# elcritch/figdraw

Hardware: AMD Instinct MI355X
Metric: Mpixels/s composited @3840x2160, 300 SDF rects+shadows; % HBM roofline (higher is better)
Workload: dtype f32 (blur taps: u8 x f16 -> f32 MFMA); 1 GPU; S300@4K: renderlist_100 scene at 3840x2160, 300 shadowed SDF rects + full-frame and 360x240 2-pass Gaussian backdrop blur(18) (BASELINE.json configs[2]); draws=707, phases=3, blur_nodes=2, fragments=41088819, parallelism=single GPU, frames_in_flight_per_gpu=4, walk_pool_threads=7, walk_pool_threads_default=7

## Files before the change

figdraw_amd/context.py:

```python
from __future__ import annotations

import ctypes as C
import os
import subprocess
from typing import Optional

import numpy as np

from . import scene as S

_HERE = os.path.dirname(os.path.abspath(__file__))
LIB_PATH = os.path.join(_HERE, "libfigdraw_hip.so")
_lib = None

_F4 = C.c_float * 4
_F2 = C.c_float * 2
_COL4 = S.CColor * 4


class FigdrawHipError(RuntimeError):
    def __init__(self, code: int, msg: str):
        super().__init__(f"[{code}] {msg}")
        self.code = code

# ... 376 lines not shown
    L.fdh_set_ui_scale.argtypes = [vp, C.c_float]
    L.fdh_render_frame.argtypes = [vp, vp, C.c_float, C.c_float, C.c_int, _F4]
    L.fdh_set_stripe.argtypes = [vp, C.c_int, C.c_int]
    L.fdh_set_blur_route.argtypes = [vp, C.c_int]
    L.fdh_set_cull.argtypes = [vp, C.c_int]
    L.fdh_culled_draws.argtypes = [vp, C.POINTER(C.c_int64)]
    L.fdh_set_walk_threads.argtypes = [vp, C.c_int]
    L.fdh_debug_host_times.argtypes = [vp, C.POINTER(C.c_int64)]
    L.fdh_walk_stats.argtypes = [vp, C.POINTER(C.c_int), C.POINTER(C.c_int64)]
    L.fdh_stripe_rows.argtypes = [C.c_int, C.c_int, C.c_int, C.POINTER(C.c_int), C.POINTER(C.c_int)]
    L.fdh_comm_unique_id.argtypes = [C.c_char_p]
    L.fdh_comm_init.argtypes = [vp, C.c_char_p, C.c_int, C.c_int]
    L.fdh_comm_destroy.argtypes = [vp]
    L.fdh_comm_share.argtypes = [vp, vp]
    L.fdh_gather_stripes.argtypes = [vp, C.c_int, vp]
    L.fdh_gather_frames.argtypes = [vp, C.c_int, C.POINTER(vp)]
    L.fdh_replay.argtypes = [vp, C.c_int]
    L.fdh_replay_async.argtypes = [vp, C.c_int]
    L.fdh_replay_timed.argtypes = [vp, C.c_int, C.POINTER(C.c_float)]
    L.fdh_profile.argtypes = [vp, C.c_int]
    L.fdh_get_frame_stats.argtypes = [vp, C.POINTER(FrameStats)]
    if hasattr(L, "fdh_block_wave_bins"):
        L.fdh_block_wave_bins.argtypes = [vp, C.POINTER(C.c_int)]
    if hasattr(L, "fdh_set_damage_tracking"):
        L.fdh_set_damage_tracking.argtypes = [vp, C.c_int]
        L.fdh_damage_bins.argtypes = [vp, vp, C.c_int, C.POINTER(C.c_int), C.POINTER(C.c_int), C.POINTER(C.c_int)]
        L.fdh_damage_changed_bins.argtypes = [vp, vp, C.c_int, C.POINTER(C.c_int), C.POINTER(C.c_int), C.POINTER(C.c_int)]
        L.fdh_damage_closure.argtypes = [vp, C.c_int, C.c_int, vp, vp, C.c_int, vp]
    if hasattr(L, "fdh_set_damage_readback"):
        L.fdh_set_damage_readback.argtypes = [vp, C.c_int]
        L.fdh_read_damage.argtypes = [vp, C.POINTER(vp), C.POINTER(vp), C.POINTER(C.c_int), C.POINTER(C.c_int), C.POINTER(C.c_int), C.POINTER(C.c_int)]
        L.fdh_read_damage_into.argtypes = [vp, vp, C.c_int64, C.c_int, C.c_int, C.POINTER(C.c_int)]
        L.fdh_apply_damage.argtypes = [vp, C.c_int64, C.c_int, C.c_int, vp, vp, C.c_int]
    if hasattr(L, "fdh_read_damage_coded"):
        L.fdh_read_damage_coded.argtypes = [vp, C.POINTER(vp), C.POINTER(vp), C.POINTER(C.c_int), C.POINTER(C.c_int64), C.POINTER(C.c_int), C.POINTER(C.c_int),
                                            C.POINTER(C.c_int)]
        L.fdh_decode_damage.argtypes = [vp, C.c_int64, C.c_int, C.c_int, vp, C.c_int, vp, C.c_int64]
        L.fdh_coded_damage_bound.argtypes = [C.c_int, C.c_int]
        L.fdh_coded_damage_bound.restype = C.c_int64
    if hasattr(L, "fdh_set_damage_exact"):
        L.fdh_set_damage_exact.argtypes = [vp, C.c_int]
        L.fdh_damage_exact_stats.argtypes = [vp, C.POINTER(C.c_int), C.POINTER(C.c_int), C.POINTER(C.c_int)]
    if hasattr(L, "fdh_read_damage_moved"):
        L.fdh_read_damage_moved.argtypes = [vp, vp, C.c_int, C.POINTER(vp), C.POINTER(vp), C.POINTER(C.c_int), C.POINTER(C.c_int64), C.POINTER(C.c_int),
                                            C.POINTER(C.c_int), C.POINTER(C.c_int), C.POINTER(C.c_int)]
        L.fdh_decode_damage_moved.argtypes = [vp, C.c_int64, C.c_int, C.c_int, vp, C.c_int, vp, C.c_int64]
# ... 775 lines not shown
    def gather_frames(self, dst_rank: int = 0, dst_ptrs=None):
        arr = (C.c_void_p * len(dst_ptrs))(*dst_ptrs) if dst_ptrs else None
        self._ck(self.L.fdh_gather_frames(self.h, int(dst_rank), arr))

    def replay(self, times: int = 1):
        self._ck(self.L.fdh_replay(self.h, int(times)))

    def replay_async(self, times: int = 1):
        self._ck(self.L.fdh_replay_async(self.h, int(times)))

    def replay_timed(self, times: int):
        out = (C.c_float * int(times))()
        self._ck(self.L.fdh_replay_timed(self.h, int(times), out))
        return np.array(out, dtype=np.float32)

    def profile(self, times: int = 1):
        self._ck(self.L.fdh_profile(self.h, int(times)))

    def frame_stats(self) -> FrameStats:
        st = FrameStats()
        self._ck(self.L.fdh_get_frame_stats(self.h, C.byref(st)))
        return st

    def block_wave_bins(self) -> int:
        n = C.c_int(0)
        self._ck(self.L.fdh_block_wave_bins(self.h, C.byref(n)))
        return n.value
```

figdraw_amd/csrc/fdh_capi.cpp:

```cpp
#include <string>

#include "fdh_context.h"
#include "fdh_damage.h"
#include "../../include/figdraw_hip_damage.h"
#include "../../include/figdraw_hip_pick.h"
#include "../../include/figdraw_hip_readback.h"
#include "../../include/figdraw_hip_stream.h"
#include "../../include/figdraw_hip_exact.h"
#include "../../include_schedule/figdraw_hip_schedule.h"
#include "../../include_readback/figdraw_hip_moves.h"
#include "../../include_glyphs/figdraw_hip_glyphs.h"
#include "../../include_glyphs/figdraw_hip_coverage.h"
#include "../../include_glyphs/figdraw_hip_cubic.h"
#include "../../include_glyphs/figdraw_hip_image_sdf.h"
#include "../../include_glyphs/figdraw_hip_device_image.h"
#include "../../include_glyphs/figdraw_hip_device_images.h"
#include "../../include_glyphs/figdraw_hip_video_frame.h"
#include "../../include_glyphs/figdraw_hip_atlas.h"
#include "../../include_video/figdraw_hip_video_out.h"
#include "../../include_video/figdraw_hip_video_planar.h"
#include "../../include_video/figdraw_hip_video_422.h"
#include "../../include_video/figdraw_hip_video_alpha.h"

using fdh::Context;
// ... 482 lines not shown
    if (!out_ns) throw fdh::Error(FDH_ERR_INVALID, "null output");
    for (int i = 0; i < 12; i++) out_ns[i] = C(c)->host_ns_[i];
  });
}
int fdh_set_walk_threads(FdhContext* c, int n) { return guard([&] { C(c)->set_walk_threads(n); }); }
int fdh_walk_stats(FdhContext* c, int* threads, int64_t* parallel_groups) {
  return guard([&] {
    if (threads) *threads = C(c)->walk_threads();
    if (parallel_groups) *parallel_groups = C(c)->parallel_groups();
  });
}
int fdh_culled_draws(FdhContext* c, int64_t* out) {
  return guard([&] {
    if (!out) throw fdh::Error(FDH_ERR_INVALID, "null output");
    *out = C(c)->culled_draws();
  });
}
int fdh_replay(FdhContext* c, int times) { return guard([&] { C(c)->replay(times); }); }
int fdh_replay_async(FdhContext* c, int times) { return guard([&] { C(c)->replay_async(times); }); }
int fdh_replay_timed(FdhContext* c, int times, float* ms_out) { return guard([&] { C(c)->replay_timed(times, ms_out); }); }
int fdh_profile(FdhContext* c, int times) { return guard([&] { C(c)->profile(times); }); }
int fdh_get_frame_stats(FdhContext* c, FdhFrameStats* out) { return guard([&] { C(c)->frame_stats(out); }); }
int fdh_block_wave_bins(FdhContext* c, int* out) { return guard([&] { *out = C(c)->block_wave_bins(); }); }

}
```

figdraw_amd/csrc/fdh_context.cpp:

```cpp
#include "fdh_context.h"
#include "fdh_host.h"
#include "fdh_walkpool.h"

#include <chrono>

#include <algorithm>
#include <cmath>
#include <cstdio>
#include <cstring>

namespace fdh {

void hip_check(hipError_t e, const char* what) {
  if (e != hipSuccess) throw Error(FDH_ERR_HIP, std::string(what) + ": " + hipGetErrorString(e));
}

void poison_fresh(void* p, size_t bytes) {
#if defined(FDH_POISON)
  if (!p || !bytes) return;
  (void)hipMemset(p, FDH_POISON, bytes);
  (void)hipDeviceSynchronize();
#else
  (void)p; (void)bytes;
#endif
// ... 427 lines not shown
  const bool big = ph.blur == J.big_blur;
  const int vy0 = std::max(j.y0, row_lo), vy1 = std::min(j.y1, row_hi);
  if (vy1 <= vy0 || j.x1 <= j.x0) return cur;
  BlurParams bp;
  bp.W = J.W; bp.H = J.H; bp.pitch = J.W;
  bp.taps = j.taps;
  bp.node_pixels = (long long)(j.x1 - j.x0) * (j.y1 - j.y0);
  bp.fuse_draw = -1;
  bp.mx_w = (size_t)ph.blur < J.mx_w_h.size() ? J.mx_w_h[ph.blur] : nullptr;
  bp.opaque = J.opaque ? 1 : 0;
  bp.x0 = j.x0; bp.x1 = j.x1; bp.y0 = vy0; bp.y1 = vy1;
  if ((size_t)ph.blur < J.blur_fused.size() && J.blur_fused[ph.blur]) {
    uint32_t* other = cur == fb_ ? alt_ : fb_;
    bp.src = cur; bp.dst = other;
    bp.fuse_draw = j.fuse_draw;
    span_begin(kSpanBlurFused);
    const bool done = launch_blur_fused(stream_, bp, J.mx_w_v[ph.blur], J.dv.recs, J.dv.exts);
    span_end();
    if (!done) throw Error(FDH_ERR_HIP, "fused blur: no kernel for this filter width (blur_fused_supported out of step with the launcher)");
    return other;
  }
  if (j.fuse_draw < 0 && J.latency_routes && blur_one_kernel_ok(j.x1 - j.x0, j.y1 - j.y0, j.taps.reach)) {
    bp.src = cur; bp.dst = backdrop_;
    span_begin(big ? kSpanBigBlurV : kSpanBlurV);
    launch_blur_small(stream_, bp);
    span_end();
    return cur;
  }
  bp.src = cur; bp.dst = blur_tmp_;
  bp.y0 = std::max(0, vy0 - j.taps.reach); bp.y1 = std::min(J.H, vy1 + j.taps.reach);
  const bool guard = partial && j.fuse_draw >= 0;
  if (guard) damage_.guard(stream_, J, ph.blur, false, cur, vy0, vy1);
  span_begin(big ? kSpanBigBlurH : kSpanBlurH);
  launch_blur_h(stream_, bp);
  span_end();
  bp.src = blur_tmp_; bp.dst = j.fuse_draw >= 0 ? cur : backdrop_;
  bp.mx_w = (size_t)ph.blur < J.mx_w_v.size() ? J.mx_w_v[ph.blur] : nullptr;
  bp.fuse_draw = j.fuse_draw;
  bp.y0 = vy0; bp.y1 = vy1;
  span_begin(big ? kSpanBigBlurV : kSpanBlurV);
  launch_blur_v(stream_, bp, J.dv.recs, J.dv.exts);
  span_end();
  if (guard) damage_.guard(stream_, J, ph.blur, true, cur, vy0, vy1);
  return cur;
}

// ... 271 lines not shown
```

figdraw_amd/csrc/fdh_context.h:

```cpp
#pragma once
#include <hip/hip_runtime.h>

#include <algorithm>
#include <atomic>
#include <chrono>
#include <condition_variable>
#include <cstdint>
#include <cstdlib>
#include <cstring>
#include <exception>
#include <memory>
#include <mutex>
#include <stdexcept>
#include <string>
#include <thread>
#include <unordered_map>
#include <vector>

#include "../../include/figdraw_hip.h"
#include "../../include/figdraw_hip_pick.h"
#include "../../include/figdraw_hip_readback.h"
#include "../../include/figdraw_hip_stream.h"
#include "fdh_kernels.h"
#include "fdh_plain.h"
// ... 115 lines not shown
  void set_pick_tag(int32_t z, int32_t id) { set_tag(PickTag{z, id}); }
  void pick_points(const float* xy, int n, int threshold, uint32_t flags, int max_hits, FdhPickHit* out, int* counts);
  void pick_region(int x, int y, int w, int h, int threshold, uint32_t flags, int32_t* out_draw);
  void pick_draw_tags(int32_t* zlevels, int32_t* ids, int cap, int* n);
  void set_cull(int mode) { frame_env_.cull_mode = mode < 0 ? 0 : (mode > 2 ? 2 : mode); }
  int64_t culled_draws() const { return culled_total_; }
  void set_walk_threads(int n) { walk_threads_ = n < 0 ? -1 : (n > 64 ? 64 : n); }
  int walk_threads() const;
  int64_t parallel_groups() const { return parallel_groups_; }
  struct GroupCuts { int first_item = -1, n = 0; std::vector<int> cut; std::vector<float> cost; uint64_t used = 0; };
  std::vector<GroupCuts>& group_cuts() { return group_cuts_; }
  void count_parallel_group() { parallel_groups_++; }
  bool may_fork() const { return env_.frame_begun && !call_log_.on(); }
  RecordedFrame& frame() { return frame_; }
  void reopen_piece() { set_phase_floor(frame_.open_piece()); }
  Recorder& pool_recorder(int slot);
  void use_device_here() const;
  void set_blur_route(int route) { blur_route_ = route < 0 ? -1 : (route ? 1 : 0); }
  void replay(int times);
  void replay_timed(int times, float* ms_out);
  void replay_async(int times);
  void profile(int times);
  int block_wave_bins() { drain(); return block_wave_bins_; }
  void frame_stats(FdhFrameStats* out) { drain(); *out = stats_; out->ms_host_launch = launch_ms_.load(std::memory_order_relaxed); }
  void flush() { drain(); }

 private:
  void release_device_state();
  void make_rect_image() override;
  void blur_node(const DrawRec& quad, const float rect[4], float blur_radius) override;
  uint32_t resolve_lcd(uint32_t flags) const {
    if (!(flags & FDH_GLYPH_LCD_CONTEXT) || (flags & FDH_GLYPH_MTSDF)) return flags;
    return (flags & ~(uint32_t)(FDH_GLYPH_LCD_FILTER | FDH_GLYPH_LCD_CONTEXT)) | (text_lcd_filtering_ ? FDH_GLYPH_LCD_FILTER : 0u);
  }
  struct FoldGuard {
    BinRec* br = nullptr;
    BBox box{0, 0, 0, 0};
    FoldGuard() = default;
    FoldGuard(FoldGuard&& o) noexcept : br(o.br), box(o.box) { o.br = nullptr; }
    FoldGuard(const FoldGuard&) = delete;
    FoldGuard& operator=(const FoldGuard&) = delete;
    ~FoldGuard() { if (br) br->box = box; }
  };

  void prepare(LaunchJob& J);
  void describe_frame(LaunchJob& J);
// ... 93 lines not shown
  bool pick_on_ = false;
  void pick_check(const char* who, int threshold, uint32_t flags);
  DeviceBuf<uint8_t> d_pick_, d_pick_spill_;
  PinnedBuf<uint8_t> h_pick_;
  int order_read_ = 0, order_nb_ = 0;
  bool order_valid_ = false;
  struct MxTables { int reach; std::vector<float> dense; std::vector<uint8_t> h, v; bool keeps_opaque = false; };
  std::vector<MxTables> mx_cache_;
  static constexpr int kStaging = RecordedFrame::kStaging;
  std::vector<std::unique_ptr<Recorder>> pool_recs_;
  HostVec<uint8_t> misc_[kStaging];
  std::vector<uint8_t> misc_host_;
  const uint8_t* misc_dev_[kStaging] = {};
  const uint8_t* misc_dev_host_[kStaging] = {};
  std::vector<uint8_t> shadow_;
  FrameLayout shadow_layout_;
  const void* shadow_dev_ = nullptr;
  int64_t uploaded_bytes_ = 0;
  hipEvent_t staging_ev_[kStaging] = {};
  char staging_busy_[kStaging] = {};
  uint32_t staging_seq_[kStaging] = {};
  volatile uint32_t* deep_host_ = nullptr;
  int block_wave_bins_ = -1;
  volatile uint32_t* seq_host_ = nullptr;
  uint32_t upload_seq_ = 0;
  void wait_staging(int slot);

  Atlas atlas_;
  GlyphMaker glyphs_;

  FdhFrameStats stats_ = {};
 public:
  int64_t host_ns_[12] = {};
  struct HostTimer {
    int64_t& acc; std::chrono::steady_clock::time_point t0;
    explicit HostTimer(int64_t& a) : acc(a), t0(std::chrono::steady_clock::now()) {}
    ~HostTimer() { acc += std::chrono::duration_cast<std::chrono::nanoseconds>(std::chrono::steady_clock::now() - t0).count(); }
  };
 private:
  std::chrono::steady_clock::time_point t_begin_frame_, t_walk_begin_;
  float host_record_ms_ = 0.0f;
};

template <typename Buf> void Context::reserve_quiet(Buf& buf, size_t n) {
  if (n <= buf.cap) return;
  drain();
  FDH_HIP(hipStreamSynchronize(stream_));
  buf.reserve(n);
}

void record_host_form(DrawRec& r);
void stripe_rows(int height, int world, int rank, int* y0, int* y1);
void comm_unique_id(uint8_t out[FDH_COMM_ID_BYTES]);
void blur_weight_fragments(float blur_radius, bool vertical, float* dense, uint16_t* frag_bits, int* reach, int* k_steps);
void saturated_core_of(const float rect[4], const float rx[4], const float ry[4], int mode, float factor, float spread,
                       const float shape[2], float aa, int out[4]);
int saturated_core_union_of(const float rect[4], const float rx[4], const float ry[4], int mode, float factor, float spread,
                            const float shape[2], float aa, int push, int out[12]);
int binrec_core_rects(const BinRec& br, int out[12]);

}
```

figdraw_amd/csrc/fdh_device.h:

```cpp
#pragma once
#include <hip/hip_runtime.h>
#include <hip/hip_ext.h>
#include <stdint.h>
#include <algorithm>
#include <type_traits>

#include "fdh_kernels.h"

#include <cstddef>
#include <cstdlib>

namespace fdh {

#ifndef FDH_STATS
#define FDH_STATS 0
#endif
#ifndef FDH_ABLATE_SHADE
#define FDH_ABLATE_SHADE 0
#endif
#ifndef FDH_TIMING
#define FDH_TIMING 0
#endif
#ifndef FDH_SPLIT_UNIFORM
#define FDH_SPLIT_UNIFORM 0
// ... 518 lines not shown
__device__ __forceinline__ void local_x4(const DrawRec& r, float cx0, float (&lx)[4]) {
  lx[0] = __builtin_fmaf(cx0 - r.ox, r.inv_w, -0.5f) * (2.0f * r.p0);
  lx[1] = lx[0] + r.kx;
  lx[2] = __builtin_fmaf(2.0f, r.kx, lx[0]);
  lx[3] = __builtin_fmaf(3.0f, r.kx, lx[0]);
}
__device__ __forceinline__ float local_y_up(const DrawRec& r, float cy) {
  return __builtin_fmaf(r.oy - cy, r.inv_h, 0.5f) * (2.0f * r.p1);
}
__device__ __forceinline__ float cover_aa(float d, float aa) { return clamp01(__builtin_fmaf(-d, aa, 0.5f)); }

__device__ __forceinline__ void unpack2(uint32_t c, f2& rg, f2& ba) {
  rg.x = (float)(c & 255u);
  rg.y = (float)((c >> 8) & 255u);
  ba.x = (float)((c >> 16) & 255u);
  ba.y = (float)(c >> 24);
}
__device__ __forceinline__ uint32_t pack2(f2 rg, f2 ba) {
  uint32_t o = __builtin_amdgcn_cvt_pk_u8_f32(rg.x, 0, 0u);
  o = __builtin_amdgcn_cvt_pk_u8_f32(rg.y, 1, o);
  o = __builtin_amdgcn_cvt_pk_u8_f32(ba.x, 2, o);
  return __builtin_amdgcn_cvt_pk_u8_f32(ba.y, 3, o);
}
}
```

figdraw_amd/csrc/fdh_kernels.h:

```cpp
#pragma once
#include <hip/hip_runtime.h>

#include <cstddef>
#include <cstdlib>

#include "fdh_types.h"

namespace fdh {

struct BinParams {
  const BinRec* binrec;
  const uint32_t* binbox;
  const uint32_t* chunkbox;
  int n_draws, binbox_shift;
  uint2* lists;
  uint32_t* counts;
  const int* phase_first;
  int n_phases, bins_x, bins_y, stride;
  const DrawRec* draws;
  const QuadExt* exts;
  int refine;
  uint32_t* seq_out = nullptr;
  uint32_t seq = 0;
  static constexpr int kBinSubs = 8;
  int sub_n = 0;
  int sub_first[kBinSubs + 1] = {};
  int sub_x0[kBinSubs] = {}, sub_y0[kBinSubs] = {}, sub_nx[kBinSubs] = {};
};

// ... 13 lines not shown
  const uint32_t* backdrop;
  int has_masks;
  int has_slow;
  int has_slow_atlas = 0;
  int has_rot;
  int has_atlas;
  int block_k8 = -1;
  uint32_t* mask_spill;
  size_t spill_stride;
  AtlasView atlas;
  int direct = 0, direct_first = 0, direct_n = 0;
  int block_max = 0;
  const BinRec* binrec = nullptr;
  int deep_k8 = 0;
  int deep_strip_min = 0;
  int deep_min = 0;
  int opaque = 0;
  uint32_t* deep_out = nullptr;
};
static_assert(offsetof(CompositeParams, deep_out) == offsetof(CompositeParams, opaque) + 4 && offsetof(CompositeParams, deep_out) + 8 == sizeof(CompositeParams), "`opaque` sits in what was padding");
static_assert(offsetof(CompositeParams, mask_spill) == offsetof(CompositeParams, block_k8) + 4 && offsetof(CompositeParams, binrec) == offsetof(CompositeParams, block_max) + 4 &&
              sizeof(CompositeParams) == 312, "`block_k8` and `block_max` sit in what was padding");

struct BlurParams {
  const uint32_t* src;
  uint32_t* dst;
  int W, H, pitch;
  int x0, y0, x1, y1;
  int fuse_draw;
  const uint4* mx_w;
  BlurTaps taps;
  long long node_pixels = 0;
  int opaque = 0;
};

void set_launch_events(hipEvent_t start, hipEvent_t stop);
bool launch_events_used();
void launch_bin(hipStream_t s, const BinParams& P);
inline int forced_kernel_paths() { static const int v = [] { const char* e = std::getenv("FDH_FORCE_KERNEL_PATHS"); return e ? std::atoi(e) : 0; }(); return v; }
struct CompositeBuild { int paths = 4; size_t lds = 0; int deep_k8 = 0; bool deep = false; bool block = false; int block_k8 = 0; };
CompositeBuild composite_build(CompositeParams& P);
void launch_composite(hipStream_t s, const DrawRec* draws, const QuadExt* exts, CompositeParams P);
void launch_blur_h(hipStream_t s, const BlurParams& P);
void launch_blur_v(hipStream_t s, const BlurParams& P, const DrawRec* draws, const QuadExt* exts);
bool blur_one_kernel_ok(int w, int h, int reach);
void launch_blur_small(hipStream_t s, const BlurParams& P);
bool blur_fused_supported(int reach, int W, int pitch);
bool launch_blur_fused(hipStream_t s, const BlurParams& P, const uint4* w_v, const DrawRec* draws, const QuadExt* exts);
void launch_fill(hipStream_t s, uint32_t* p, uint32_t v, size_t n);
void launch_rasterize_lines(hipStream_t s, const float4* lines, int n, int w, int h, float* scratch, uint32_t* out);
void launch_lcd_filter(hipStream_t s, const uint32_t* src, uint32_t* dst, int w, int h);
void launch_minify2(hipStream_t s, const uint32_t* src, uint32_t* dst, int sw, int sh);
void launch_atlas_blit(hipStream_t s, uint32_t* level, int LS, int x, int y, const uint32_t* src, int w, int h);
void launch_msdf_generate(hipStream_t s, const float* edges, int n_edges, int w, int h, float orient, float range, uint32_t* out);
void launch_msdf_correct(hipStream_t s, const float* edges, int n_edges, int w, int h, float orient, float range, const uint32_t* in, uint32_t* out);
void launch_msdf_generate_union(hipStream_t s, const float* edges, int n_edges, int w, int h, float orient, float range, uint32_t* out);
void launch_msdf_correct_union(hipStream_t s, const float* edges, int n_edges, int w, int h, float orient, float range, const uint32_t* in, uint32_t* out);
// ... 51 lines not shown
```

figdraw_amd/csrc/fdh_prepare.cpp:

```cpp
#include "fdh_context.h"
#include "fdh_damage.h"
#include "fdh_host.h"

#include <algorithm>
#include <chrono>
#include <cmath>
#include <cstring>

namespace fdh {

static uint16_t half_bits_rne(float f) {
  uint32_t u;
  std::memcpy(&u, &f, 4);
  const uint16_t sign = (uint16_t)((u >> 16) & 0x8000u);
  const float a = std::fabs(f);
  if (a == 0.0f) return sign;
  std::memcpy(&u, &a, 4);
  const int e = (int)(u >> 23) - 127;
  if (e < -14) return sign | (uint16_t)std::nearbyint(a * 16777216.0f);
  const uint32_t mant = u & 0x7fffffu, m = mant >> 13, rem = mant & 0x1fffu;
  uint32_t h = ((uint32_t)(e + 15) << 10) | m;
  if (rem > 0x1000u || (rem == 0x1000u && (m & 1u))) h++;
  return sign | (uint16_t)h;
}
// ... 21 lines not shown
  float q[2 * kMaxBlurReach + 1];
  quantise_taps_f16(t, q);
  double sum[32] = {};
  for (int m = 0; m < nk; m++)
    for (int lane = 0; lane < 64; lane++) {
      const int j = lane & 31, g = lane >> 5;
      for (int e = 0; e < 8; e++) {
        const int k = 16 * m + mx_krow(g, e, vertical) - delta - j;
#if FDH_MX_LO
        const float w = (k >= 0 && k <= 2 * t.reach) ? t.dense[kBlurPad + k] * 1024.0f : 0.0f;
        const uint16_t hi = half_bits_rne(w), lo = half_bits_rne(w - half_value(hi));
#else
        const float w = (k >= 0 && k <= 2 * t.reach) ? q[k] : 0.0f;
        const uint16_t hi = half_bits_rne(w), lo = 0;
#endif
        o[(((size_t)(2 * m) * 64 + lane) * 8) + e] = hi;
        o[(((size_t)(2 * m + 1) * 64 + lane) * 8) + e] = lo;
        sum[j] += (double)half_value(hi) + (double)half_value(lo);
      }
    }
  double dev = 0.0;
  for (int j = 0; j < 32; j++) dev = std::max(dev, std::fabs(sum[j] - 1024.0));
  return (float)dev;
}

void blur_weight_fragments(float blur_radius, bool vertical, float* dense, uint16_t* frag_bits, int* reach, int* k_steps) {
  const BlurTaps t = make_taps(blur_radius);
  for (int k = 0; k <= 2 * t.reach; k++) dense[k] = t.dense[kBlurPad + k];
  *reach = t.reach;
  *k_steps = mx_nk(t.reach, vertical);
  if (*k_steps > kMxMaxNK) throw Error(FDH_ERR_INVALID, "blur_weight_fragments: filter too wide");
  build_mx_weights(t, vertical, reinterpret_cast<uint8_t*>(frag_bits));
}

void FrameLayout::lay_out(size_t n_recs, size_t n_exts, size_t n_phases, const std::vector<BlurJob>& blurs) {
  n = n_recs; n_ext = n_exts;
  n_chunks = std::max<size_t>((n + 255) / 256, 1);
  recs = 0;
  exts = align256(recs + n * sizeof(DrawRec));
  binrecs = align256(exts + n_ext * sizeof(QuadExt));
  boxes = align256(binrecs + n * sizeof(BinRec));
  chunks = align256(boxes + ((n + 3) & ~(size_t)3) * sizeof(uint32_t));
  phase_first = align256(chunks + n_chunks * sizeof(uint32_t));
  tables = align256(phase_first + (n_phases + 1) * sizeof(int));
  total = tables;
  mx_h.assign(blurs.size(), 0); mx_v.assign(blurs.size(), 0);
// ... 377 lines not shown
```

figdraw_amd/csrc/k_blur_valu.hip:

```cpp
#include "fdh_device.h"

namespace fdh {
bool launch_blur_mx_pass(bool vertical, hipStream_t s, const BlurParams& P, const DrawRec* draws, const QuadExt* exts);


template <int kBlurOut, int kUnroll = 1, typename Tex>
__device__ __forceinline__ void fir_outputs(const float* __restrict__ d, int reach, Tex tex, f2 (&rg)[kBlurOut], f2 (&ba)[kBlurOut]) {
#pragma unroll
  for (int p = 0; p < kBlurOut; p++) { rg[p] = 0.0f; ba[p] = 0.0f; }
  const int nwin = kBlurOut + 2 * reach;
#pragma unroll
  for (int j = 0; j < kBlurOut - 1; j++) {
    f2 trg, tba;
    unpack2(tex(j), trg, tba);
#pragma unroll
    for (int p = 0; p <= j; p++) {
      const float c = d[j - p + kBlurPad];
      rg[p] += trg * c;
      ba[p] += tba * c;
    }
  }
#pragma unroll kUnroll
  for (int j = kBlurOut - 1; j < nwin - (kBlurOut - 1); j++) {
    f2 trg, tba;
    unpack2(tex(j), trg, tba);
#pragma unroll
    for (int p = 0; p < kBlurOut; p++) {
      const float c = d[j - p + kBlurPad];
      rg[p] += trg * c;
      ba[p] += tba * c;
    }
  }
#pragma unroll
  for (int i = kBlurOut - 2; i >= 0; i--) {
    const int j = nwin - 1 - i;
    f2 trg, tba;
    unpack2(tex(j), trg, tba);
#pragma unroll
    for (int p = kBlurOut - 1 - i; p < kBlurOut; p++) {
      const float c = d[j - p + kBlurPad];
      rg[p] += trg * c;
      ba[p] += tba * c;
    }
  }
}

template <int kBlurOut>
__global__ __launch_bounds__(256) void k_blur_h(BlurParams P) {
  constexpr int kBlurHW = 64 * kBlurOut;
  constexpr int kBlurHLine = kBlurHW + 2 * kMaxBlurReach + kBlurOut;
  __shared__ __attribute__((aligned(16))) uint32_t lines[4][kBlurHLine];
  const int wave = threadIdx.x >> 6, lane = threadIdx.x & 63;
  const int y = P.y0 + blockIdx.y * 4 + wave;
  const int xs = P.x0 + blockIdx.x * kBlurHW;
  const int reach = P.taps.reach;
  const int wpx = min(kBlurHW, P.x1 - xs);
  const int span = wpx + 2 * reach;
  uint32_t* line = lines[wave];
  if (y < P.y1) {
    const uint32_t* __restrict__ row = P.src + (size_t)y * P.pitch;
    if (xs - reach >= 0 && xs - reach + span + kBlurOut <= P.W) {
      const uint32_t* __restrict__ p = row + (xs - reach);
      for (int i = lane; i < span + kBlurOut; i += 64) line[i] = p[i];
    } else {
      for (int i = lane; i < span + kBlurOut; i += 64) {
        int x = xs - reach + i;
        x = x < 0 ? 0 : (x > P.W - 1 ? P.W - 1 : x);
        line[i] = row[x];
      }
// ... 76 lines not shown
  for (int p = 0; p < kBlurOut; p++) {
    if (y + p >= P.y1) break;
    const size_t pix = (size_t)(y + p) * P.pitch + x;
    float alpha = 1.0f;
    if (!core) {
      const Frag f = make_frag(r, exts, x, y + p);
      if (!f.covered) continue;
      const float lx = (f.u - 0.5f) * 2.0f * r.p0, ly = (f.v - 0.5f) * 2.0f * r.p1;
      const float dist = shape_dist((r.op_mode & F_ELLIP) != 0u, lx, -ly, r.p2, r.p3, r.r[0], r.r[1], r.r[2], r.r[3]);
      alpha = 1.0f - clamp01(r.aa * dist + 0.5f);
    }
    if (__all(__builtin_rintf(ba[p].y) == 255.0f && alpha == 1.0f)) {
      P.dst[pix] = pack2(rg[p], ba[p]);
      continue;
    }
    const F4 b = {__builtin_rintf(rg[p].x), __builtin_rintf(rg[p].y), __builtin_rintf(ba[p].x), __builtin_rintf(ba[p].y)};
    F4 F = unpack255(P.dst[pix]);
    const float sa = b.w * k * alpha, A = 255.0f * sa;
    const f2 brg = {b.x, b.y};
    blend_pre(F, brg * k * A, f2{b.z * k * A, A}, 1.0f - sa);
    P.dst[pix] = pack255(F);
  }
}

constexpr int kSmallTW = 16, kSmallTH = 24, kSmallHOut = 2, kSmallVOut = 2, kSmallThreads = 1024;
__global__ __launch_bounds__(kSmallThreads) void k_blur_small(BlurParams P) {
  extern __shared__ uint32_t small_lds[];
#if FDH_TIMING
  const unsigned long long W_in = wall_clock64();
  unsigned long long W_asked = 0, W_staged = 0, W_h = 0, W_hb = 0, W_v = 0;
#endif
  const int reach = P.taps.reach;
  const int in_w = kSmallTW + 2 * reach, rows = kSmallTH + 2 * reach;
  uint32_t* in = small_lds;
  uint32_t* hres = small_lds + rows * in_w;
  const int ntx = (P.x1 - P.x0 + kSmallTW - 1) / kSmallTW;
  const int ty = (int)blockIdx.x / ntx, tx = (int)blockIdx.x - ty * ntx;
  const int xs = P.x0 + tx * kSmallTW, ys = P.y0 + ty * kSmallTH;
  constexpr int kSmallStage = 5;
  const int n_in = rows * in_w;
  uint32_t texel[kSmallStage];
  const bool by_rows = in_w <= 64 && rows <= kSmallStage * (kSmallThreads / 64);
  if (by_rows) {
    const int wv = (int)threadIdx.x >> 6, ln = (int)threadIdx.x & 63;
    int x = xs - reach + min(ln, in_w - 1);
    x = x < 0 ? 0 : (x > P.W - 1 ? P.W - 1 : x);
#pragma unroll
    for (int k = 0; k < kSmallStage; k++) {
      int y = ys - reach + min(wv + k * (kSmallThreads / 64), rows - 1);
      y = y < 0 ? 0 : (y > P.H - 1 ? P.H - 1 : y);
// ... 15 lines not shown
#endif
  if (by_rows) {
    const int wv = (int)threadIdx.x >> 6, ln = (int)threadIdx.x & 63;
#pragma unroll
    for (int k = 0; k < kSmallStage; k++) {
      const int rr = wv + k * (kSmallThreads / 64);
      if (ln < in_w && rr < rows) in[rr * in_w + ln] = texel[k];
    }
  } else {
#pragma unroll
    for (int k = 0; k < kSmallStage; k++) {
      const int i = (int)threadIdx.x + k * kSmallThreads;
      if (i < n_in) in[i] = texel[k];
    }
  }
  __syncthreads();
#if FDH_TIMING
  W_staged = wall_clock64();
#endif
  for (int t = threadIdx.x; t < rows * (kSmallTW / kSmallHOut); t += kSmallThreads) {
    const int rr = t / (kSmallTW / kSmallHOut), c = t - rr * (kSmallTW / kSmallHOut);
    f2 rg[kSmallHOut], ba[kSmallHOut];
    const uint32_t* __restrict__ win = in + rr * in_w + kSmallHOut * c;
    fir_outputs<kSmallHOut, 6>(P.taps.dense, reach, [&](int j) { return win[j]; }, rg, ba);
#pragma unroll
    for (int o = 0; o < kSmallHOut; o++) hres[rr * kSmallTW + kSmallHOut * c + o] = pack2(rg[o], ba[o]);
  }
#if FDH_TIMING
  W_h = wall_clock64();
#endif
  __syncthreads();
#if FDH_TIMING
  W_hb = wall_clock64();
#endif
  for (int t = threadIdx.x; t < kSmallTW * (kSmallTH / kSmallVOut); t += kSmallThreads) {
    const int pr = t / kSmallTW, c = t - pr * kSmallTW;
    const int x = xs + c, y = ys + kSmallVOut * pr;
    if (x >= P.x1 || y >= P.y1) continue;
    f2 rg[kSmallVOut], ba[kSmallVOut];
    const uint32_t* __restrict__ col = hres + (kSmallVOut * pr) * kSmallTW + c;
    fir_outputs<kSmallVOut, 6>(P.taps.dense, reach, [&](int j) { return col[j * kSmallTW]; }, rg, ba);
#pragma unroll
    for (int o = 0; o < kSmallVOut; o++)
      if (y + o < P.y1) P.dst[(size_t)(y + o) * P.pitch + x] = pack2(rg[o], ba[o]);
  }
#if FDH_TIMING
  W_v = wall_clock64();
  if ((threadIdx.x & 63) == 0 && blockIdx.x < 2048) {
    unsigned long long* row = g_wave_times + 16 * ((size_t)blockIdx.x * 16 + (threadIdx.x >> 6));
    row[1] = W_in; row[2] = W_asked; row[3] = W_staged; row[4] = W_h; row[5] = W_hb; row[7] = W_v; row[6] = 8;
  }
#endif
}

constexpr int kBlurVWaves = 4;
static bool blur_small(const BlurParams& P) {
  if (blur_forced_path()) return blur_forced_path() == 1;
  return (P.node_pixels > 0 ? P.node_pixels : (long long)(P.x1 - P.x0) * (P.y1 - P.y0)) < 384 * 1024;
}
static int blur_pick_nout(int extent, int quantum, int reach) {
  int best = 8;
  double best_cost = 1e300;
  for (int n : {8, 10, 12}) {
    const int unit = quantum * n;
    const double padded = (double)((extent + unit - 1) / unit) * unit;
    const double per_output = 2.0 * (2 * reach + 1) + 4.0 * (n + 2 * reach) / n + 6.0;
    const double cost = padded * per_output;
    if (cost < best_cost) { best_cost = cost; best = n; }
  }
  return best;
}
template <int NOUT> static void launch_blur_h_n(hipStream_t s, const BlurParams& P) {
  dim3 grid((P.x1 - P.x0 + 64 * NOUT - 1) / (64 * NOUT), (P.y1 - P.y0 + 3) / 4);
  FDH_LAUNCH(k_blur_h<NOUT>, grid, dim3(256), 0, s, P);
}
template <int NOUT, int WAVES> static void launch_blur_v_n(hipStream_t s, const BlurParams& P, const DrawRec* draws, const QuadExt* exts) {
  const int ntx = (P.x1 - P.x0 + kBlurVW - 1) / kBlurVW, nty = (P.y1 - P.y0 + WAVES * NOUT - 1) / (WAVES * NOUT);
  dim3 grid(8 * ((ntx * nty + 7) / 8));
  const size_t lds = (size_t)(WAVES * NOUT + 2 * P.taps.reach) * kBlurVW * sizeof(uint32_t);
  FDH_LAUNCH((k_blur_v<NOUT, WAVES>), grid, dim3(64 * WAVES), lds, s, P, draws, exts);
}
bool blur_one_kernel_ok(int w, int h, int reach) {
  if (blur_forced_path() || w <= 0 || h <= 0) return false;
  return (long long)w * h < 384 * 1024 && reach <= 24;
}
void launch_blur_small(hipStream_t s, const BlurParams& P) {
  if (P.x1 <= P.x0 || P.y1 <= P.y0) return;
  const int reach = P.taps.reach, ntx = (P.x1 - P.x0 + kSmallTW - 1) / kSmallTW, nty = (P.y1 - P.y0 + kSmallTH - 1) / kSmallTH;
  const size_t lds = (size_t)(kSmallTH + 2 * reach) * (size_t)(2 * kSmallTW + 2 * reach) * sizeof(uint32_t);
  FDH_LAUNCH(k_blur_small, dim3(ntx * nty), dim3(kSmallThreads), lds, s, P);
}
void launch_blur_h(hipStream_t s, const BlurParams& P) {
  if (P.x1 <= P.x0 || P.y1 <= P.y0) return;
  if (blur_small(P)) { launch_blur_h_n<2>(s, P); return; }
  if (blur_forced_path() != 2 && launch_blur_mx_pass(false, s, P, nullptr, nullptr)) return;
  switch (blur_pick_nout(P.x1 - P.x0, 64, P.taps.reach)) {
    case 12: launch_blur_h_n<12>(s, P); break;
    case 10: launch_blur_h_n<10>(s, P); break;
    case 16: launch_blur_h_n<16>(s, P); break;
    default: launch_blur_h_n<8>(s, P); break;
  }
}
void launch_blur_v(hipStream_t s, const BlurParams& P, const DrawRec* draws, const QuadExt* exts) {
  if (P.x1 <= P.x0 || P.y1 <= P.y0) return;
  if (blur_small(P)) { launch_blur_v_n<2, 4>(s, P, draws, exts); return; }
  if (blur_forced_path() != 2 && launch_blur_mx_pass(true, s, P, draws, exts)) return;
  switch (blur_pick_nout(P.y1 - P.y0, kBlurVWaves, P.taps.reach)) {
    case 12: launch_blur_v_n<12, kBlurVWaves>(s, P, draws, exts); break;
    case 10: launch_blur_v_n<10, kBlurVWaves>(s, P, draws, exts); break;
    case 16: launch_blur_v_n<16, kBlurVWaves>(s, P, draws, exts); break;
    default: launch_blur_v_n<8, kBlurVWaves>(s, P, draws, exts); break;
  }
}
}
```

include_schedule/figdraw_hip_schedule.h:

```cpp
#ifndef FIGDRAW_HIP_SCHEDULE_H
#define FIGDRAW_HIP_SCHEDULE_H
#include "../include/figdraw_hip.h"

#ifdef __cplusplus
extern "C" {
#endif

FDH_API int fdh_block_wave_bins(FdhContext*, int* out);

#ifdef __cplusplus
}
#endif
#endif
```

Baseline: 207,800 Mpixels/s.

## Skip alpha channel in small blur when opaque; add tall-tile small blur variant

Templates the single-kernel small blur on an opaque flag. When the source is opaque and the normalized taps provably keep alpha at 255 through both passes, the kernel skips alpha unpack and FMA and writes 0xFF directly. It also adds a taller-tile variant (512 threads, 4 outputs per thread, staged row loads), selected only by an environment variable. The opaque check runs on the host per blur and reports its result through a new query API. This trims VALU work on the 360x240 blur node, which is a small part of the frame.

```diff
diff --git a/figdraw_amd/context.py b/figdraw_amd/context.py
--- a/figdraw_amd/context.py
+++ b/figdraw_amd/context.py
@@ -422,6 +422,9 @@
     L.fdh_get_frame_stats.argtypes = [vp, C.POINTER(FrameStats)]
     if hasattr(L, "fdh_block_wave_bins"):
         L.fdh_block_wave_bins.argtypes = [vp, C.POINTER(C.c_int)]
+    if hasattr(L, "fdh_small_blur_form"):
+        L.fdh_small_blur_form.argtypes = [vp, C.POINTER(C.c_int)]
+        L.fdh_blur_small_alpha_sums.argtypes = [C.POINTER(C.c_float), C.c_int, C.POINTER(C.c_float), C.POINTER(C.c_int)]
     if hasattr(L, "fdh_set_damage_tracking"):
         L.fdh_set_damage_tracking.argtypes = [vp, C.c_int]
         L.fdh_damage_bins.argtypes = [vp, vp, C.c_int, C.POINTER(C.c_int), C.POINTER(C.c_int), C.POINTER(C.c_int)]
@@ -1243,6 +1246,11 @@
         self._ck(self.L.fdh_get_frame_stats(self.h, C.byref(st)))
         return st
 
+    def small_blur_form(self) -> int:
+        n = C.c_int(0)
+        self._ck(self.L.fdh_small_blur_form(self.h, C.byref(n)))
+        return n.value
+
     def block_wave_bins(self) -> int:
         n = C.c_int(0)
         self._ck(self.L.fdh_block_wave_bins(self.h, C.byref(n)))
diff --git a/figdraw_amd/csrc/fdh_blur_params.h b/figdraw_amd/csrc/fdh_blur_params.h
--- /dev/null
+++ b/figdraw_amd/csrc/fdh_blur_params.h
@@ -0,0 +1,24 @@
+#pragma once
+#if defined(__HIP__) || defined(__HIPCC__)
+#include <hip/hip_runtime.h>
+#endif
+#include <stdint.h>
+
+#include "fdh_types.h"
+
+namespace fdh {
+
+struct BlurParams {
+  const uint32_t* src;
+  uint32_t* dst;
+  int W, H, pitch;
+  int x0, y0, x1, y1;
+  int fuse_draw;
+  const uint4* mx_w;
+  BlurTaps taps;
+  long long node_pixels = 0;
+  int opaque = 0;
+  int small_tall = 0;
+};
+
+}
diff --git a/figdraw_amd/csrc/fdh_capi.cpp b/figdraw_amd/csrc/fdh_capi.cpp
--- a/figdraw_amd/csrc/fdh_capi.cpp
+++ b/figdraw_amd/csrc/fdh_capi.cpp
@@ -528,5 +528,12 @@
 int fdh_profile(FdhContext* c, int times) { return guard([&] { C(c)->profile(times); }); }
 int fdh_get_frame_stats(FdhContext* c, FdhFrameStats* out) { return guard([&] { C(c)->frame_stats(out); }); }
 int fdh_block_wave_bins(FdhContext* c, int* out) { return guard([&] { *out = C(c)->block_wave_bins(); }); }
-
-}
+int fdh_small_blur_form(FdhContext* c, int* out) { return guard([&] { *out = C(c)->small_blur_form(); }); }
+int fdh_blur_small_alpha_sums(const float* dense, int reach, float sums[2], int* keeps_opaque) {
+  return guard([&] {
+    if (!dense || !sums || !keeps_opaque || reach < 0 || reach > fdh::kMaxBlurReach) throw fdh::Error(FDH_ERR_INVALID, "fdh_blur_small_alpha_sums: null pointer or reach out of range");
+    *keeps_opaque = fdh::blur_taps_keep_opaque(dense, reach, sums) ? 1 : 0;
+  });
+}
+
+}
diff --git a/figdraw_amd/csrc/fdh_context.cpp b/figdraw_amd/csrc/fdh_context.cpp
--- a/figdraw_amd/csrc/fdh_context.cpp
+++ b/figdraw_amd/csrc/fdh_context.cpp
@@ -473,6 +473,10 @@
   }
   if (j.fuse_draw < 0 && J.latency_routes && blur_one_kernel_ok(j.x1 - j.x0, j.y1 - j.y0, j.taps.reach)) {
     bp.src = cur; bp.dst = backdrop_;
+    bp.opaque = J.opaque && blur_taps_keep_opaque(j.taps.dense + kBlurPad, j.taps.reach, nullptr) ? 1 : 0;
+    static const int form_env = [] { const char* e = std::getenv("FDH_SMALL_BLUR_FORM"); return e ? std::atoi(e) : 0; }();
+    bp.small_tall = form_env == 1 || (form_env == 2 && device_shared_now(device_, this)) ? 1 : 0;
+    small_blur_form_ = bp.small_tall | (bp.opaque << 1);
     span_begin(big ? kSpanBigBlurV : kSpanBlurV);
     launch_blur_small(stream_, bp);
     span_end();
diff --git a/figdraw_amd/csrc/fdh_context.h b/figdraw_amd/csrc/fdh_context.h
--- a/figdraw_amd/csrc/fdh_context.h
+++ b/figdraw_amd/csrc/fdh_context.h
@@ -161,6 +161,7 @@
   void replay_async(int times);
   void profile(int times);
   int block_wave_bins() { drain(); return block_wave_bins_; }
+  int small_blur_form() { drain(); return small_blur_form_; }
   void frame_stats(FdhFrameStats* out) { drain(); *out = stats_; out->ms_host_launch = launch_ms_.load(std::memory_order_relaxed); }
   void flush() { drain(); }
 
@@ -300,6 +301,7 @@
   uint32_t staging_seq_[kStaging] = {};
   volatile uint32_t* deep_host_ = nullptr;
   int block_wave_bins_ = -1;
+  int small_blur_form_ = -1;
   volatile uint32_t* seq_host_ = nullptr;
   uint32_t upload_seq_ = 0;
   void wait_staging(int slot);
@@ -331,6 +333,7 @@
 void stripe_rows(int height, int world, int rank, int* y0, int* y1);
 void comm_unique_id(uint8_t out[FDH_COMM_ID_BYTES]);
 void blur_weight_fragments(float blur_radius, bool vertical, float* dense, uint16_t* frag_bits, int* reach, int* k_steps);
+bool blur_taps_keep_opaque(const float* dense, int reach, float sums[2]);
 void saturated_core_of(const float rect[4], const float rx[4], const float ry[4], int mode, float factor, float spread,
                        const float shape[2], float aa, int out[4]);
 int saturated_core_union_of(const float rect[4], const float rx[4], const float ry[4], int mode, float factor, float spread,
diff --git a/figdraw_amd/csrc/fdh_device.h b/figdraw_amd/csrc/fdh_device.h
--- a/figdraw_amd/csrc/fdh_device.h
+++ b/figdraw_amd/csrc/fdh_device.h
@@ -564,4 +564,14 @@
   o = __builtin_amdgcn_cvt_pk_u8_f32(ba.x, 2, o);
   return __builtin_amdgcn_cvt_pk_u8_f32(ba.y, 3, o);
 }
-}
+__device__ __forceinline__ void unpack2_opaque(uint32_t c, f2& rg, f2& ba) {
+  rg.x = (float)(c & 255u);
+  rg.y = (float)((c >> 8) & 255u);
+  ba.x = (float)((c >> 16) & 255u);
+}
+__device__ __forceinline__ uint32_t pack2_opaque(f2 rg, f2 ba) {
+  uint32_t o = __builtin_amdgcn_cvt_pk_u8_f32(rg.x, 0, 0xFF000000u);
+  o = __builtin_amdgcn_cvt_pk_u8_f32(rg.y, 1, o);
+  return __builtin_amdgcn_cvt_pk_u8_f32(ba.x, 2, o);
+}
+}
diff --git a/figdraw_amd/csrc/fdh_kernels.h b/figdraw_amd/csrc/fdh_kernels.h
--- a/figdraw_amd/csrc/fdh_kernels.h
+++ b/figdraw_amd/csrc/fdh_kernels.h
@@ -5,6 +5,7 @@
 #include <cstdlib>
 
 #include "fdh_types.h"
+#include "fdh_blur_params.h"
 
 namespace fdh {
 
@@ -64,17 +65,6 @@
 static_assert(offsetof(CompositeParams, mask_spill) == offsetof(CompositeParams, block_k8) + 4 && offsetof(CompositeParams, binrec) == offsetof(CompositeParams, block_max) + 4 &&
               sizeof(CompositeParams) == 312, "`block_k8` and `block_max` sit in what was padding");
 
-struct BlurParams {
-  const uint32_t* src;
-  uint32_t* dst;
-  int W, H, pitch;
-  int x0, y0, x1, y1;
-  int fuse_draw;
-  const uint4* mx_w;
-  BlurTaps taps;
-  long long node_pixels = 0;
-  int opaque = 0;
-};
 
 void set_launch_events(hipEvent_t start, hipEvent_t stop);
 bool launch_events_used();
diff --git a/figdraw_amd/csrc/fdh_prepare.cpp b/figdraw_amd/csrc/fdh_prepare.cpp
--- a/figdraw_amd/csrc/fdh_prepare.cpp
+++ b/figdraw_amd/csrc/fdh_prepare.cpp
@@ -67,6 +67,23 @@
   double dev = 0.0;
   for (int j = 0; j < 32; j++) dev = std::max(dev, std::fabs(sum[j] - 1024.0));
   return (float)dev;
+}
+
+bool blur_taps_keep_opaque(const float* dense, int reach, float sums[2]) {
+  float fused = 255.0f, plain = 255.0f;
+  bool keeps = true;
+  for (int stage = 0; stage < 2; stage++) {
+    float a = 0.0f, b = 0.0f;
+    for (int k = 0; k <= 2 * reach; k++) {
+      a = std::fmaf(fused, dense[k], a);
+      volatile float prod = plain * dense[k];
+      b = b + prod;
+    }
+    if (sums) sums[stage] = a;
+    fused = std::nearbyintf(a); plain = std::nearbyintf(b);
+    keeps = keeps && fused == 255.0f && plain == 255.0f;
+  }
+  return keeps;
 }
 
 void blur_weight_fragments(float blur_radius, bool vertical, float* dense, uint16_t* frag_bits, int* reach, int* k_steps) {
diff --git a/figdraw_amd/csrc/k_blur_valu.hip b/figdraw_amd/csrc/k_blur_valu.hip
--- a/figdraw_amd/csrc/k_blur_valu.hip
+++ b/figdraw_amd/csrc/k_blur_valu.hip
@@ -1,10 +1,19 @@
 #include "fdh_device.h"
+#ifndef FDH_BLUR_SMALL_ALONE
+#define FDH_BLUR_SMALL_ALONE 0
+#endif
 
 namespace fdh {
 bool launch_blur_mx_pass(bool vertical, hipStream_t s, const BlurParams& P, const DrawRec* draws, const QuadExt* exts);
 
 
-template <int kBlurOut, int kUnroll = 1, typename Tex>
+template <int kCh> __device__ __forceinline__ void fir_unpack(uint32_t c, f2& rg, f2& ba) {
+  if constexpr (kCh == 4) unpack2(c, rg, ba); else unpack2_opaque(c, rg, ba);
+}
+template <int kCh> __device__ __forceinline__ uint32_t fir_pack(f2 rg, f2 ba) {
+  if constexpr (kCh == 4) return pack2(rg, ba); else return pack2_opaque(rg, ba);
+}
+template <int kBlurOut, int kUnroll = 1, int kCh = 4, typename Tex>
 __device__ __forceinline__ void fir_outputs(const float* __restrict__ d, int reach, Tex tex, f2 (&rg)[kBlurOut], f2 (&ba)[kBlurOut]) {
 #pragma unroll
   for (int p = 0; p < kBlurOut; p++) { rg[p] = 0.0f; ba[p] = 0.0f; }
@@ -12,39 +21,40 @@
 #pragma unroll
   for (int j = 0; j < kBlurOut - 1; j++) {
     f2 trg, tba;
-    unpack2(tex(j), trg, tba);
+    fir_unpack<kCh>(tex(j), trg, tba);
 #pragma unroll
     for (int p = 0; p <= j; p++) {
       const float c = d[j - p + kBlurPad];
       rg[p] += trg * c;
-      ba[p] += tba * c;
+      if constexpr (kCh == 4) ba[p] += tba * c; else ba[p].x += tba.x * c;
     }
   }
 #pragma unroll kUnroll
   for (int j = kBlurOut - 1; j < nwin - (kBlurOut - 1); j++) {
     f2 trg, tba;
-    unpack2(tex(j), trg, tba);
+    fir_unpack<kCh>(tex(j), trg, tba);
 #pragma unroll
     for (int p = 0; p < kBlurOut; p++) {
       const float c = d[j - p + kBlurPad];
       rg[p] += trg * c;
-      ba[p] += tba * c;
+      if constexpr (kCh == 4) ba[p] += tba * c; else ba[p].x += tba.x * c;
     }
   }
 #pragma unroll
   for (int i = kBlurOut - 2; i >= 0; i--) {
     const int j = nwin - 1 - i;
     f2 trg, tba;
-    unpack2(tex(j), trg, tba);
+    fir_unpack<kCh>(tex(j), trg, tba);
 #pragma unroll
     for (int p = kBlurOut - 1 - i; p < kBlurOut; p++) {
       const float c = d[j - p + kBlurPad];
       rg[p] += trg * c;
-      ba[p] += tba * c;
-    }
-  }
-}
-
+      if constexpr (kCh == 4) ba[p] += tba * c; else ba[p].x += tba.x * c;
+    }
+  }
+}
+
+#if !FDH_BLUR_SMALL_ALONE
 template <int kBlurOut>
 __global__ __launch_bounds__(256) void k_blur_h(BlurParams P) {
   constexpr int kBlurHW = 64 * kBlurOut;
@@ -167,10 +177,13 @@
     P.dst[pix] = pack255(F);
   }
 }
+#endif
 
 constexpr int kSmallTW = 16, kSmallTH = 24, kSmallHOut = 2, kSmallVOut = 2, kSmallThreads = 1024;
+template <bool kOpaque>
 __global__ __launch_bounds__(kSmallThreads) void k_blur_small(BlurParams P) {
-  extern __shared__ uint32_t small_lds[];
+  HIP_DYNAMIC_SHARED(uint32_t, small_lds)
+  constexpr int kCh = kOpaque ? 3 : 4;
 #if FDH_TIMING
   const unsigned long long W_in = wall_clock64();
   unsigned long long W_asked = 0, W_staged = 0, W_h = 0, W_hb = 0, W_v = 0;
@@ -232,9 +245,9 @@
     const int rr = t / (kSmallTW / kSmallHOut), c = t - rr * (kSmallTW / kSmallHOut);
     f2 rg[kSmallHOut], ba[kSmallHOut];
     const uint32_t* __restrict__ win = in + rr * in_w + kSmallHOut * c;
-    fir_outputs<kSmallHOut, 6>(P.taps.dense, reach, [&](int j) { return win[j]; }, rg, ba);
-#pragma unroll
-    for (int o = 0; o < kSmallHOut; o++) hres[rr * kSmallTW + kSmallHOut * c + o] = pack2(rg[o], ba[o]);
+    fir_outputs<kSmallHOut, 6, kCh>(P.taps.dense, reach, [&](int j) { return win[j]; }, rg, ba);
+#pragma unroll
+    for (int o = 0; o < kSmallHOut; o++) hres[rr * kSmallTW + kSmallHOut * c + o] = fir_pack<kCh>(rg[o], ba[o]);
   }
 #if FDH_TIMING
   W_h = wall_clock64();
@@ -249,10 +262,10 @@
     if (x >= P.x1 || y >= P.y1) continue;
     f2 rg[kSmallVOut], ba[kSmallVOut];
     const uint32_t* __restrict__ col = hres + (kSmallVOut * pr) * kSmallTW + c;
-    fir_outputs<kSmallVOut, 6>(P.taps.dense, reach, [&](int j) { return col[j * kSmallTW]; }, rg, ba);
+    fir_outputs<kSmallVOut, 6, kCh>(P.taps.dense, reach, [&](int j) { return col[j * kSmallTW]; }, rg, ba);
 #pragma unroll
     for (int o = 0; o < kSmallVOut; o++)
-      if (y + o < P.y1) P.dst[(size_t)(y + o) * P.pitch + x] = pack2(rg[o], ba[o]);
+      if (y + o < P.y1) P.dst[(size_t)(y + o) * P.pitch + x] = fir_pack<kCh>(rg[o], ba[o]);
   }
 #if FDH_TIMING
   W_v = wall_clock64();
@@ -263,6 +276,87 @@
 #endif
 }
 
+constexpr int kTallOut = 4, kTallThreads = 512, kTallStage = 8;
+template <bool kOpaque>
+__global__ __launch_bounds__(kTallThreads) void k_blur_small_tall(BlurParams P, int th) {
+  HIP_DYNAMIC_SHARED(uint32_t, small_lds)
+  constexpr int kCh = kOpaque ? 3 : 4;
+  constexpr int kWaves = kTallThreads / 64;
+  const int reach = P.taps.reach;
+  const int ntx = (P.x1 - P.x0 + kSmallTW - 1) / kSmallTW;
+  const int ty = (int)blockIdx.x / ntx, tx = (int)blockIdx.x - ty * ntx;
+  const int xs = P.x0 + tx * kSmallTW, ys = P.y0 + ty * th;
+  const int th_here = min(th, (P.y1 - ys + kTallOut - 1) & ~(kTallOut - 1));
+  const int in_w = kSmallTW + 2 * reach, rows = th_here + 2 * reach;
+  uint32_t* in = small_lds;
+  uint32_t* hres = small_lds + rows * in_w;
+  {
+    const int wv = (int)threadIdx.x >> 6, ln = (int)threadIdx.x & 63;
+    int x = xs - reach + min(ln, in_w - 1);
+    x = x < 0 ? 0 : (x > P.W - 1 ? P.W - 1 : x);
+    for (int r0 = wv; r0 < rows; r0 += kWaves * kTallStage) {
+      uint32_t texel[kTallStage];
+#pragma unroll
+      for (int k = 0; k < kTallStage; k++) {
+        int y = ys - reach + min(r0 + k * kWaves, rows - 1);
+        y = y < 0 ? 0 : (y > P.H - 1 ? P.H - 1 : y);
+        texel[k] = P.src[(size_t)y * P.pitch + x];
+      }
+#pragma unroll
+      for (int k = 0; k < kTallStage; k++) {
+        const int rr = r0 + k * kWaves;
+        if (ln < in_w && rr < rows) in[rr * in_w + ln] = texel[k];
+      }
+    }
+  }
+  __syncthreads();
+  for (int t = threadIdx.x; t < rows * (kSmallTW / kTallOut); t += kTallThreads) {
+    const int rr = t / (kSmallTW / kTallOut), c = t - rr * (kSmallTW / kTallOut);
+    f2 rg[kTallOut], ba[kTallOut];
+    const uint32_t* __restrict__ win = in + rr * in_w + kTallOut * c;
+    fir_outputs<kTallOut, 4, kCh>(P.taps.dense, reach, [&](int j) { return win[j]; }, rg, ba);
+#pragma unroll
+    for (int o = 0; o < kTallOut; o++) hres[rr * kSmallTW + kTallOut * c + o] = fir_pack<kCh>(rg[o], ba[o]);
+  }
+  __syncthreads();
+  for (int t = threadIdx.x; t < kSmallTW * (th_here / kTallOut); t += kTallThreads) {
+    const int pr = t / kSmallTW, c = t - pr * kSmallTW;
+    const int x = xs + c, y = ys + kTallOut * pr;
+    if (x >= P.x1 || y >= P.y1) continue;
+    f2 rg[kTallOut], ba[kTallOut];
+    const uint32_t* __restrict__ col = hres + (kTallOut * pr) * kSmallTW + c;
+    fir_outputs<kTallOut, 4, kCh>(P.taps.dense, reach, [&](int j) { return col[j * kSmallTW]; }, rg, ba);
+#pragma unroll
+    for (int o = 0; o < kTallOut; o++)
+      if (y + o < P.y1) P.dst[(size_t)(y + o) * P.pitch + x] = fir_pack<kCh>(rg[o], ba[o]);
+  }
+}
+
+constexpr int kSmallTallTH = 60;
+static int small_tall_th(int reach) {
+  static const int env = [] { const char* e = std::getenv("FDH_SMALL_BLUR_TH"); return e ? std::atoi(e) : 0; }();
+  int th = env > 0 ? env : kSmallTallTH;
+  th = (th < kTallOut ? kTallOut : (th > 128 ? 128 : th)) & ~(kTallOut - 1);
+  const int most = ((40 * 1024 / 4 - 1) / (2 * kSmallTW + 2 * reach) - 2 * reach) & ~(kTallOut - 1);
+  return th < most ? th : most;
+}
+void launch_blur_small(hipStream_t s, const BlurParams& P) {
+  if (P.x1 <= P.x0 || P.y1 <= P.y0) return;
+  const int reach = P.taps.reach, ntx = (P.x1 - P.x0 + kSmallTW - 1) / kSmallTW;
+  if (P.small_tall) {
+    const int th = small_tall_th(reach), nty = (P.y1 - P.y0 + th - 1) / th;
+    const size_t lds = (size_t)(th + 2 * reach) * (size_t)(2 * kSmallTW + 2 * reach) * sizeof(uint32_t);
+    if (P.opaque) FDH_LAUNCH(k_blur_small_tall<true>, dim3(ntx * nty), dim3(kTallThreads), lds, s, P, th);
+    else FDH_LAUNCH(k_blur_small_tall<false>, dim3(ntx * nty), dim3(kTallThreads), lds, s, P, th);
+    return;
+  }
+  const int nty = (P.y1 - P.y0 + kSmallTH - 1) / kSmallTH;
+  const size_t lds = (size_t)(kSmallTH + 2 * reach) * (size_t)(2 * kSmallTW + 2 * reach) * sizeof(uint32_t);
+  if (P.opaque) FDH_LAUNCH(k_blur_small<true>, dim3(ntx * nty), dim3(kSmallThreads), lds, s, P);
+  else FDH_LAUNCH(k_blur_small<false>, dim3(ntx * nty), dim3(kSmallThreads), lds, s, P);
+}
+
+#if !FDH_BLUR_SMALL_ALONE
 constexpr int kBlurVWaves = 4;
 static bool blur_small(const BlurParams& P) {
   if (blur_forced_path()) return blur_forced_path() == 1;
@@ -294,12 +388,6 @@
   if (blur_forced_path() || w <= 0 || h <= 0) return false;
   return (long long)w * h < 384 * 1024 && reach <= 24;
 }
-void launch_blur_small(hipStream_t s, const BlurParams& P) {
-  if (P.x1 <= P.x0 || P.y1 <= P.y0) return;
-  const int reach = P.taps.reach, ntx = (P.x1 - P.x0 + kSmallTW - 1) / kSmallTW, nty = (P.y1 - P.y0 + kSmallTH - 1) / kSmallTH;
-  const size_t lds = (size_t)(kSmallTH + 2 * reach) * (size_t)(2 * kSmallTW + 2 * reach) * sizeof(uint32_t);
-  FDH_LAUNCH(k_blur_small, dim3(ntx * nty), dim3(kSmallThreads), lds, s, P);
-}
 void launch_blur_h(hipStream_t s, const BlurParams& P) {
   if (P.x1 <= P.x0 || P.y1 <= P.y0) return;
   if (blur_small(P)) { launch_blur_h_n<2>(s, P); return; }
@@ -322,4 +410,5 @@
     default: launch_blur_v_n<8, kBlurVWaves>(s, P, draws, exts); break;
   }
 }
-}
+#endif
+}
diff --git a/include_schedule/figdraw_hip_schedule.h b/include_schedule/figdraw_hip_schedule.h
--- a/include_schedule/figdraw_hip_schedule.h
+++ b/include_schedule/figdraw_hip_schedule.h
@@ -8,6 +8,9 @@
 
 FDH_API int fdh_block_wave_bins(FdhContext*, int* out);
 
+FDH_API int fdh_small_blur_form(FdhContext*, int* out);
+FDH_API int fdh_blur_small_alpha_sums(const float* dense, int reach, float sums[2], int* keeps_opaque);
+
 #ifdef __cplusplus
 }
 #endif
```

Measured after the change: 208,900 Mpixels/s (median of 6 runs). Within noise of the previous version (+0.5%).
